# jafarinia/snuffy

Measured on AMD Instinct MI355X. Metric: slides/sec, higher is better.
Workload: dtype f32; 1 GPU; cfgB: MILNet eval forward, 1 bag/step/rank, N=32768 patches D=768 h=6 Lambda=200 (K=200) depth=1 relu mlp x4; parallelism=bag-parallel x1, bags_resident_per_rank=8, launch=hip graph replay, rccl_ranks=0

## Files before the change

### include/snuffy_hip.h

```cpp
#ifndef SNUFFY_HIP_H
#define SNUFFY_HIP_H

#include <stddef.h>
#include <stdint.h>

#ifdef __cplusplus
extern "C" {
#endif

typedef void* snf_stream_t;

#define SNF_OK 0
#define SNF_EINVAL (-1)
#define SNF_ELAUNCH (-2)
#define SNF_EUNSUPPORTED (-3)
#define SNF_EWORKSPACE (-4)

#define SNF_ACT_RELU 0
#define SNF_ACT_GELU 1
#define SNF_ACT_LEAKYRELU 2
#define SNF_ACT_SELU 3
#define SNF_ACT_NONE 4

#define SNF_DT_F32 0
// ... 171 lines not shown
int snf_gemm_bf16_resid_f32(const void* a, int64_t lda, const void* w, int64_t ldw, const float* bias, const float* resid, int64_t ldr,
                            int64_t m, int n, int k, int act, float* c, int64_t ldc, int tile_n, snf_stream_t stream);
int snf_gemm_bf16_lnfold(const void* a, int64_t lda, const void* w, int64_t ldw, const float* colsum, const float* bias,
                         const float* rowstats, int64_t m, int n, int k, int act, void* c, int64_t ldc, snf_stream_t stream);
int snf_gemm_bf16_resid(const void* a, int64_t lda, const void* w, int64_t ldw, const float* bias, int64_t m, int n, int k, float* x,
                        int64_t ldx, void* x_bf16, int64_t ldxb, float* stats_part, snf_stream_t stream);
int snf_gemm_hl_bf16(const void* a_hl, int64_t lda, const void* w_hl, int64_t ldw, const float* bias, int64_t m, int n, int k,
                     int act, void* c, int64_t ldc, int out_dtype, snf_stream_t stream);
int snf_gemm_hl_resid_bf16(const void* a_hl, int64_t lda, const void* w_hl, int64_t ldw, const float* bias, const float* resid,
                           int64_t ldr, int64_t m, int n, int k, int act, void* c, int64_t ldc, int out_dtype, snf_stream_t stream);
size_t snf_gemm_hl_ws_bytes(int64_t m, int n, int k);
int snf_gemm_hl_gated_bf16(const void* a_hl, int64_t lda, const void* w_hl, int64_t ldw, const void* gate_hl, int64_t ldg, int64_t m, int n,
                           int k, void* c_hl, int64_t ldc, snf_stream_t stream);
size_t snf_gemm_tn_ws_bytes(int64_t n, int p, int q);
int snf_gemm_tn_f32(const void* a, int64_t lda, int a_hi, int a_lo, const void* b, int64_t ldb, int b_hi, int b_lo, int hl, int64_t n, int p,
                    int q, float* c, int64_t ldc, void* workspace, size_t workspace_bytes, snf_stream_t stream);
int snf_gemm_hl_ws_bf16(const void* a_hl, int64_t lda, const void* w_hl, int64_t ldw, const float* bias, const float* resid,
                        int64_t ldr, int64_t m, int n, int k, int act, void* c, int64_t ldc, int out_dtype, void* workspace,
                        size_t workspace_bytes, snf_stream_t stream);
size_t snf_gemm_hl_deferred_ws_bytes(int64_t m, int n, int k, size_t* slab_offset);
int snf_gemm_hl_deferred_f32(const void* a_hl, int64_t lda, const void* w_hl, int64_t ldw, const float* bias, const float* resid,
                             int64_t ldr, int64_t m, int n, int k, int act, float* c, int64_t ldc, int out_dtype, void* workspace,
                             size_t workspace_bytes, snf_stream_t stream);
int snf_gemm_hl_dropout_bf16(const void* a_hl, int64_t lda, const void* w_hl, int64_t ldw, const float* bias, const float* resid,
                             int64_t ldr, int64_t m, int n, int k, int act, void* c, int64_t ldc, int out_dtype, float dropout_p,
                             uint64_t seed, uint64_t offset, snf_stream_t stream);
int snf_gemm_hl_ws_dropout_bf16(const void* a_hl, int64_t lda, const void* w_hl, int64_t ldw, const float* bias, const float* resid,
                                int64_t ldr, int64_t m, int n, int k, int act, void* c, int64_t ldc, int out_dtype, float dropout_p,
                                uint64_t seed, uint64_t offset, void* workspace, size_t workspace_bytes, snf_stream_t stream);
int snf_split_hl_colsum_dropout_f32(const float* x, int64_t ldx, int64_t m, int k, const void* gate_hl, int64_t ldg, float dropout_p,
                                    uint64_t seed, uint64_t offset, void* out_hl, int64_t ldo, float* partial, snf_stream_t stream);
int snf_split_hl_f32(const float* x, int64_t ldx, int64_t m, int k, void* out_bf16, snf_stream_t stream);
int snf_layernorm_rows_hl_f32(const float* x, int64_t n, int d, const int32_t* slot_map, const float* patch_rows,
                              const float* gamma, const float* beta, float eps, void* out_bf16, snf_stream_t stream);
int snf_layernorm_rows_hl_patch_f32(const float* x, const float* addend, int64_t n, int d, const int64_t* out_row_idx,
                                    const float* gamma, const float* beta, float eps, void* out_hl, snf_stream_t stream);

int snf_vit_patchify(const float* img, int b, int c, int hgt, int wid, int patch, void* cols, int out_dtype,
                     snf_stream_t stream);
int snf_vit_assemble_tokens(const void* patch_emb, int pe_dtype, const float* cls_token, const float* pos_embed, int b,
                            int num_patches, int d, float* tokens, snf_stream_t stream);
int snf_vit_residual_ln(float* x, int64_t n, int d, const void* add1_bf16, const void* add2_bf16, float scale2,
                        const float* gamma, const float* beta, float eps, void* ln_out_bf16, void* x_bf16,
                        snf_stream_t stream);
int snf_vit_row_stats(const float* x, int64_t ldx, const float* part, int slots, int64_t n, int d, float eps, float* stats,
                      void* x_bf16, int64_t ldxb, snf_stream_t stream);
// ... 140 lines not shown
```

### snuffy_amd/_ffi.py

```python
import ctypes
import os
from ctypes import c_char_p, c_float, c_int, c_int64, c_size_t, c_uint64, c_void_p

_HERE = os.path.dirname(os.path.abspath(__file__))
LIB_PATH = os.environ.get("SNUFFY_HIP_LIB") or os.path.join(_HERE, "lib", "libsnuffy_hip.so")

SNF_OK = 0
SNF_EINVAL = -1
SNF_ELAUNCH = -2
SNF_EUNSUPPORTED = -3
SNF_EWORKSPACE = -4

ACT_CODES = {"relu": 0, "gelu": 1, "leakyrelu": 2, "selu": 3, "none": 4}
DT_F32 = 0
DT_BF16 = 1
DT_BF16_SPLIT3 = 2
DT_BF16_HL = 3
TOPK_MAX_K = 2048

SIGNATURES = {
    "snf_version": (c_char_p, []),
    "snf_last_error": (c_char_p, []),
    "snf_device_cu_count": (c_int, []),
    "snf_critic_f32": (c_int, [c_void_p, c_int64, c_int, c_void_p, c_void_p, c_int, c_void_p, c_void_p, c_void_p,
# ... 111 lines not shown
                                     c_void_p, c_int64, c_void_p]),
    "snf_gemm_bf16_resid": (c_int, [c_void_p, c_int64, c_void_p, c_int64, c_void_p, c_int64, c_int, c_int, c_void_p, c_int64, c_void_p,
                                    c_int64, c_void_p, c_void_p]),
    "snf_vit_row_stats": (c_int, [c_void_p, c_int64, c_void_p, c_int, c_int64, c_int, c_float, c_void_p, c_void_p, c_int64, c_void_p]),
    "snf_split_hl_f32": (c_int, [c_void_p, c_int64, c_int64, c_int, c_void_p, c_void_p]),
    "snf_layernorm_rows_hl_patch_f32": (c_int, [c_void_p, c_void_p, c_int64, c_int, c_void_p, c_void_p, c_void_p, c_float, c_void_p,
                                                c_void_p]),
    "snf_layernorm_rows_hl_f32": (c_int, [c_void_p, c_int64, c_int, c_void_p, c_void_p, c_void_p, c_void_p, c_float,
                                          c_void_p, c_void_p]),
    "snf_gemm_hl_resid_bf16": (c_int, [c_void_p, c_int64, c_void_p, c_int64, c_void_p, c_void_p, c_int64, c_int64, c_int, c_int, c_int,
                                       c_void_p, c_int64, c_int, c_void_p]),
    "snf_gemm_hl_ws_bytes": (c_size_t, [c_int64, c_int, c_int]),
    "snf_gemm_hl_gated_bf16": (c_int, [c_void_p, c_int64, c_void_p, c_int64, c_void_p, c_int64, c_int64, c_int, c_int, c_void_p, c_int64,
                                       c_void_p]),
    "snf_gemm_tn_ws_bytes": (c_size_t, [c_int64, c_int, c_int]),
    "snf_gemm_tn_f32": (c_int, [c_void_p, c_int64, c_int, c_int, c_void_p, c_int64, c_int, c_int, c_int, c_int64, c_int, c_int, c_void_p,
                                c_int64, c_void_p, c_size_t, c_void_p]),
    "snf_split_hl_colsum_f32": (c_int, [c_void_p, c_int64, c_int64, c_int, c_void_p, c_int64, c_void_p, c_int64, c_void_p, c_void_p]),
    "snf_gemm_hl_ws_bf16": (c_int, [c_void_p, c_int64, c_void_p, c_int64, c_void_p, c_void_p, c_int64, c_int64, c_int, c_int, c_int,
                                    c_void_p, c_int64, c_int, c_void_p, c_size_t, c_void_p]),
    "snf_gemm_hl_deferred_ws_bytes": (c_size_t, [c_int64, c_int, c_int, c_void_p]),
    "snf_gemm_hl_deferred_f32": (c_int, [c_void_p, c_int64, c_void_p, c_int64, c_void_p, c_void_p, c_int64, c_int64, c_int, c_int, c_int,
                                         c_void_p, c_int64, c_int, c_void_p, c_size_t, c_void_p]),
    "snf_gemm_bf16_dropout": (c_int, [c_void_p, c_int64, c_void_p, c_int64, c_void_p, c_int64, c_int, c_int, c_int, c_void_p, c_int64,
                                      c_int, c_int, c_float, c_uint64, c_uint64, c_void_p]),
    "snf_dropout_rows_bf16": (c_int, [c_void_p, c_int64, c_int64, c_int, c_float, c_uint64, c_uint64, c_void_p]),
    "snf_residual_assemble_dropout_f32": (c_int, [c_void_p, c_int64, c_int, c_void_p, c_void_p, c_void_p, c_void_p, c_float, c_uint64,
                                                  c_uint64, c_void_p, c_void_p]),
    "snf_colsum_fused_dropout": (c_int, [c_void_p, c_int, c_int64, c_int, c_float, c_uint64, c_uint64, c_void_p, c_void_p, c_void_p]),
    "snf_gemm_hl_dropout_bf16": (c_int, [c_void_p, c_int64, c_void_p, c_int64, c_void_p, c_void_p, c_int64, c_int64, c_int, c_int, c_int,
                                         c_void_p, c_int64, c_int, c_float, c_uint64, c_uint64, c_void_p]),
    "snf_gemm_hl_ws_dropout_bf16": (c_int, [c_void_p, c_int64, c_void_p, c_int64, c_void_p, c_void_p, c_int64, c_int64, c_int, c_int, c_int,
                                            c_void_p, c_int64, c_int, c_float, c_uint64, c_uint64, c_void_p, c_size_t, c_void_p]),
    "snf_split_hl_colsum_dropout_f32": (c_int, [c_void_p, c_int64, c_int64, c_int, c_void_p, c_int64, c_float, c_uint64, c_uint64,
                                                c_void_p, c_int64, c_void_p, c_void_p]),
    "snf_gemm_hl_bf16": (c_int, [c_void_p, c_int64, c_void_p, c_int64, c_void_p, c_int64, c_int, c_int, c_int, c_void_p, c_int64,
                                 c_int, c_void_p]),
    "snf_topk_segmented_f32": (c_int, [c_void_p, c_void_p, c_int, c_int64, c_int, c_void_p, c_void_p]),
    "snf_sparse_attn_varlen_plan": (c_int, [c_void_p, c_int, c_int, c_int, c_int, c_void_p, c_size_t, c_void_p, c_void_p]),
    "snf_sparse_attn_fwd_mfma_varlen": (c_int, [c_void_p, c_int64, c_void_p, c_int64, c_void_p, c_int, c_void_p, c_int, c_int, c_int,
                                                c_int, c_float, c_void_p, c_void_p, c_void_p, c_void_p, c_void_p, c_size_t,
                                                c_void_p]),
    "snf_sparse_attn_x3_varlen_plan": (c_int, [c_void_p, c_int, c_int, c_int, c_int, c_void_p, c_size_t, c_void_p, c_void_p]),
    "snf_sparse_attn_fwd_x3_varlen": (c_int, [c_void_p, c_int64, c_void_p, c_int64, c_void_p, c_void_p, c_int, c_int, c_int, c_int,
                                              c_float, c_void_p, c_void_p, c_void_p, c_void_p, c_void_p, c_size_t, c_void_p]),
    "snf_sparse_attn_varlen_chunked_plan": (c_int, [c_void_p, c_int, c_int, c_int, c_int, c_void_p, c_size_t, c_void_p, c_void_p,
# ... 105 lines not shown
```

### snuffy_amd/csrc/gemm.hip

```cpp
#include <stdlib.h>

#include "mfma.h"
#include "philox.h"

namespace {

struct GemmParams {
    const unsigned short* a;
    const unsigned short* w;
    const float* bias;
    void* c;
    int64_t lda, ldw, ldc;
    int m, n, k;
    int act;
    int tiles_m, tiles_n;
    unsigned long long* trace;
    const float* resid = nullptr;
    int64_t ldr = 0;
    unsigned int* split_cnt = nullptr;
    float* split_slab = nullptr;
    int split_cap = 0, split_rcap = 0;
    const unsigned short* gate = nullptr;
    int64_t ldg = 0;
    const float* colsum = nullptr;
// ... 436 lines not shown
            barrier();
        }
        bias_landed();
#ifdef SNF_GEMM_NOSTORE
        if (false) {
#else
        if (full) {
#endif
            epilogue(tile, std::true_type{});
            after_epilogue = true;
        } else {
            epilogue(tile, std::false_type{});
            wait_vmcnt<0>();
        }
        if (!has_next) break;
        tile = next;
        cur = nxt;
    }
    if (wid < 4) __builtin_amdgcn_s_barrier();
}

template <int ACT, int OUT, int SPLIT_MODE = 0, bool GATE = false, bool DROP = false>
__global__ __launch_bounds__(512, 2) void gemm_hl_kernel(GemmParams P) {
    constexpr bool SPLIT = SPLIT_MODE != 0, DEFER = SPLIT_MODE == 2;
    static_assert(!DEFER || (SPLIT && OUT == 1 && ACT == SNF_ACT_NONE && !GATE && !DROP), "gemm_hl: the deferred split writes plain fp32");
    static_assert(!GATE || (OUT == 3 && ACT == SNF_ACT_NONE && !SPLIT), "gemm_hl: the gated form writes an hl image, no activation, no split");
    static_assert(!DROP || (!GATE && (OUT == 1 || OUT == 3)), "gemm_hl: dropout goes with the fp32 and the hl-image outputs");
    constexpr int NI = 4, BN = 256;
    constexpr int ROWL = 128;
    constexpr int IMG = BM * ROWL;
    constexpr int STEP_BYTES = 2 * IMG;
    constexpr int NC = 4 * NI;
    constexpr bool LINE_STORES = (OUT == 1 || OUT == 3) && ACT != SNF_ACT_GELU && ACT != SNF_ACT_SELU;
    extern __shared__ __attribute__((aligned(16))) unsigned char smem[];

    const int lane = threadIdx.x & 63;
    const int wid = __builtin_amdgcn_readfirstlane(threadIdx.x >> 6);
    const int wr = wid >> 2, wc = wid & 3;
    const int ns_all = P.k / BKS;
    unsigned char* const scr = smem + 2 * STEP_BYTES + wid * 4096;

    const int ntiles = P.tiles_m * P.tiles_n;
    const int xcd = blockIdx.x & 7, wg_in_xcd = blockIdx.x >> 3, wgs_per_xcd = gridDim.x >> 3;
    if constexpr (!SPLIT) {
        if (P.split_cap >= 2 && blockIdx.x == 0) {
            for (int i = threadIdx.x; i < 8 * P.split_rcap; i += 512) P.split_cnt[i] = 0u;
            asm volatile("s_waitcnt vmcnt(0)" ::: "memory");
        }
    }
    int t_lo, t_hi;
    {
        const int q = ntiles >> 3, r = ntiles & 7;
        t_lo = xcd < r ? xcd * (q + 1) : r * (q + 1) + (xcd - r) * q;
        t_hi = t_lo + q + (xcd < r ? 1 : 0);
    }
    int sp_part = 0, sp_parts = 1, sp_slot = 0, sp_tile = -1;
    if (P.split_cap >= 2) {
        const int q_x = t_hi - t_lo, full_rounds = q_x / wgs_per_xcd, r = q_x - full_rounds * wgs_per_xcd;
        int sn = r > 0 ? wgs_per_xcd / r : 0;
        if (sn > P.split_cap) sn = P.split_cap;
        if (sn > ns_all / HL_SPLIT_MIN_STEPS) sn = ns_all / HL_SPLIT_MIN_STEPS;
        if (sn >= 2 && r <= P.split_rcap) {
            if constexpr (SPLIT) {
                if (wg_in_xcd < r * sn) {
                    const int jr = wg_in_xcd % r;
                    sp_tile = t_lo + full_rounds * wgs_per_xcd + jr;
                    sp_part = wg_in_xcd / r, sp_parts = sn, sp_slot = xcd * P.split_rcap + jr;
                }
            } else {
                t_hi = t_lo + full_rounds * wgs_per_xcd;
            }
        }
    }
    int tile = t_lo + wg_in_xcd;
    if constexpr (SPLIT) {
        tile = __builtin_amdgcn_readfirstlane(sp_tile);
        sp_part = __builtin_amdgcn_readfirstlane(sp_part), sp_parts = __builtin_amdgcn_readfirstlane(sp_parts);
        sp_slot = __builtin_amdgcn_readfirstlane(sp_slot);
        if (tile < 0) return;
        t_hi = tile + 1;
        asm volatile("" : "+s"(t_hi));
    } else {
        if (tile >= t_hi) return;
    }
    const int s_begin = SPLIT ? __builtin_amdgcn_readfirstlane(sp_part * ns_all / sp_parts) : 0;
    const int ns = SPLIT ? __builtin_amdgcn_readfirstlane((sp_part + 1) * ns_all / sp_parts) - s_begin : ns_all;
    const unsigned short* const a_base = P.a + (SPLIT ? s_begin * 64 : 0);
    const unsigned short* const w_base = P.w + (SPLIT ? s_begin * 64 : 0);

    struct Src {
        int a[4], w[4];
    };
    auto tile_src_mn = [&](int tm, int tn) __attribute__((always_inline)) -> Src {
        Src s;
        int ln = lane;
        asm volatile("" : "+v"(ln));
        const int c = ln & 7;
#pragma unroll
        for (int j = 0; j < 4; ++j) {
            const int row = (4 * wid + j) * 8 + (ln >> 3);
            int grow = tm * BM + row;
            if (grow > P.m - 1) grow = P.m - 1;
            s.a[j] = grow * (int)P.lda + ((c ^ ((row >> 1) & 7)) << 3);
            int wrow = tn * BN + row;
            if (wrow > P.n - 1) wrow = P.n - 1;
            s.w[j] = wrow * (int)P.ldw + ((c ^ (((row >> 1) & 1) | (((row >> 3) & 3) << 1))) << 3);
        }
        return s;
    };
// ... 21 lines not shown

    f32x4 acc[8][NI];
    bf16x8 xf[8], wh[NI], wl[NI];
    f32x4 bv4[NC / 4];

    auto frag = [&](const unsigned char* p) __attribute__((always_inline)) -> bf16x8 {
#ifdef X3_NOREAD
        u32x4 z = {1u, 2u, 3u, (unsigned)lane};
        asm volatile("" : "+v"(z));
        return __builtin_bit_cast(bf16x8, z);
#endif
        return __builtin_bit_cast(bf16x8, *reinterpret_cast<const u32x4*>(p));
    };
#ifdef X3_NOMFMA
#define X3_MFMA(a, b, c) ([&]() { f32x4 t_ = (c); asm volatile("" : "+v"(t_) : "v"(a), "v"(b)); return t_; }())
#else
#define X3_MFMA(a, b, c) __builtin_amdgcn_mfma_f32_16x16x32_bf16(a, b, c, 0, 0, 0)
#endif
    auto load_bias = [&](int tl) __attribute__((always_inline)) {
#pragma unroll
        for (int c4 = 0; c4 < NC / 4; ++c4) bv4[c4] = f32x4{0.f, 0.f, 0.f, 0.f};
        if (P.bias) {
            const int tn = tl % P.tiles_n;
            const int n0 = tn * BN + 64 * wc + 8 * fg;
            const float* bp0 = P.bias + (n0 + 8 <= P.n ? n0 : 0);
            const float* bp1 = P.bias + (n0 + 40 <= P.n ? n0 + 32 : 0);
            asm volatile("global_load_dwordx4 %0, %1, off" : "=v"(bv4[0]) : "v"(bp0) : "memory");
            asm volatile("global_load_dwordx4 %0, %1, off offset:16" : "=v"(bv4[1]) : "v"(bp0) : "memory");
            asm volatile("global_load_dwordx4 %0, %1, off" : "=v"(bv4[2]) : "v"(bp1) : "memory");
            asm volatile("global_load_dwordx4 %0, %1, off offset:16" : "=v"(bv4[3]) : "v"(bp1) : "memory");
        }
    };
    auto bias_landed = [&]() __attribute__((always_inline)) {
#pragma unroll
        for (int c4 = 0; c4 < NC / 4; ++c4) asm volatile("" : "+v"(bv4[c4]));
    };
    auto epilogue = [&](int tl, auto full_t) __attribute__((always_inline)) {
        constexpr bool FULL = decltype(full_t)::value;
        const int tm = tl / P.tiles_n, tn = tl - tm * P.tiles_n;
        const int n0 = tn * BN + 64 * wc + 8 * fg;
        const int row0 = tm * BM + 128 * wr + fi;
        int lane_o = lane;
        asm volatile("" : "+v"(lane_o));
        const int fio = lane_o & 15, fgo = lane_o >> 4;
#pragma unroll
        for (int mi = 0; mi < 8; ++mi) {
            const int row = row0 + 16 * mi;
#pragma unroll
            for (int h = 0; h < NI / 2; ++h) {
                float v[8];
#pragma unroll
                for (int e = 0; e < 8; ++e) v[e] = activate<ACT>(acc[mi][2 * h + (e >> 2)][e & 3] + bv4[2 * h + (e >> 2)][e & 3]);
                const int col = n0 + 32 * h;
                if constexpr (DROP) {
                    const snf::philox_f4 m0 = snf::dropout_mask4(P.drop, 0, P.m, row, P.n, col);
                    const snf::philox_f4 m1 = snf::dropout_mask4(P.drop, 0, P.m, row, P.n, col + 4);
#pragma unroll
                    for (int e = 0; e < 4; ++e) {
                        v[e] *= m0[e];
                        v[4 + e] *= m1[e];
                    }
#pragma unroll
                    for (int e = 0; e < 8; ++e) asm volatile("" : "+v"(v[e]));
                }
// ... 36 lines not shown
                        if (ok) *reinterpret_cast<u32x4*>(dst) = pk;
                    } else {
                        float lo[8];
#pragma unroll
                        for (int e = 0; e < 8; ++e)
                            lo[e] = v[e] - __uint_as_float((e & 1) ? (pk[e >> 1] & 0xffff0000u) : (pk[e >> 1] << 16));
                        const u32x4 pl = {cvt_pk_bf16(lo[0], lo[1]), cvt_pk_bf16(lo[2], lo[3]), cvt_pk_bf16(lo[4], lo[5]), cvt_pk_bf16(lo[6], lo[7])};
                        unsigned short* dst = reinterpret_cast<unsigned short*>(P.c) + (int64_t)row * P.ldc + 64 * (col >> 5) + (col & 31);
                        if constexpr (LINE_STORES) {
                            *reinterpret_cast<u32x4*>(scr + fio * 256 + (((8 * h + fgo) ^ fio) << 4)) = pk;
                            *reinterpret_cast<u32x4*>(scr + fio * 256 + (((8 * h + 4 + fgo) ^ fio) << 4)) = pl;
                        } else if (ok) {
                            *reinterpret_cast<u32x4*>(dst) = pk;
                            *reinterpret_cast<u32x4*>(dst + 32) = pl;
                        }
                    }
                }
            }
            if constexpr (LINE_STORES) {
                const int lr = lane_o >> 4, lc = lane_o & 15;
                unsigned char* const crow = reinterpret_cast<unsigned char*>(P.c) +
                                            (OUT == 1 ? 4 * (int64_t)(tn * BN + 64 * wc) : 2 * 2 * (int64_t)(tn * BN + 64 * wc));
                const int64_t pitch = (OUT == 1 ? 4 : 2) * P.ldc;
#pragma unroll
                for (int jj = 0; jj < 4; ++jj) {
                    const int r = lr + 4 * jj;
                    const u32x4 val = *reinterpret_cast<const u32x4*>(scr + r * 256 + ((lc ^ r) << 4));
                    const int orow = tm * BM + 128 * wr + 16 * mi + r;
                    const int ocol = tn * BN + 64 * wc + (OUT == 1 ? 4 * lc : 32 * (lc >> 3) + 8 * (lc & 3));
#ifdef X3_NOSTORE
                    const bool ok2 = val[0] == 0x12345678u && orow < 0;
#else
                    const bool ok2 = FULL || (orow < P.m && ocol + (OUT == 1 ? 4 : 8) <= P.n);
#endif
                    if (ok2) *reinterpret_cast<u32x4*>(crow + orow * pitch + 16 * lc) = val;
                }
            }
        }
    };

    Src cur = tile_src(tile);
    stage(cur, 0, 0);
    int buf = 0;
    bool after_epilogue = false;
    while (true) {
        const int next = tile + wgs_per_xcd;
        const bool has_next = next < t_hi;
        const bool full = (tile / P.tiles_n + 1) * BM <= P.m && (tile % P.tiles_n + 1) * BN <= P.n;
        for (int s = 0; s < ns; ++s) {
            if (!(s == 0 && after_epilogue)) wait_vmcnt<0>();
            after_epilogue = false;
            __builtin_amdgcn_sched_barrier(0);
            __builtin_amdgcn_s_barrier();
            __builtin_amdgcn_sched_barrier(0);
            const unsigned char* base = smem + buf * STEP_BYTES;
#pragma unroll
            for (int ni = 0; ni < NI; ++ni) wh[ni] = frag(base + woff_h + (4 * (ni & 1) + 32 * (ni >> 1)) * ROWL);
#pragma unroll
            for (int mi = 0; mi < 8; ++mi) xf[mi] = frag(base + xoff_h + mi * 16 * ROWL);
#pragma unroll
            for (int ni = 0; ni < NI; ++ni) wl[ni] = frag(base + woff_l + (4 * (ni & 1) + 32 * (ni >> 1)) * ROWL);
            __builtin_amdgcn_sched_barrier(0);
            if (s + 1 < ns) {
                stage(cur, s + 1, buf ^ 1);
            } else if (has_next) {
                cur = tile_src(next);
                stage(cur, 0, buf ^ 1);
            }
            __builtin_amdgcn_sched_barrier(0);
            __builtin_amdgcn_s_setprio(1);
            if (s == 0) {
#pragma unroll
                for (int mi = 0; mi < 8; ++mi)
#pragma unroll
                    for (int ni = 0; ni < NI; ++ni) acc[mi][ni] = X3_MFMA(wh[ni], xf[mi], (f32x4{0.f, 0.f, 0.f, 0.f}));
            } else {
#pragma unroll
                for (int mi = 0; mi < 8; ++mi)
#pragma unroll
                    for (int ni = 0; ni < NI; ++ni) acc[mi][ni] = X3_MFMA(wh[ni], xf[mi], acc[mi][ni]);
            }
#pragma unroll
            for (int mi = 0; mi < 8; ++mi) {
#pragma unroll
                for (int ni = 0; ni < NI; ++ni) acc[mi][ni] = X3_MFMA(wl[ni], xf[mi], acc[mi][ni]);
                __builtin_amdgcn_sched_barrier(0);
                xf[mi] = frag(base + xoff_l + mi * 16 * ROWL);
                __builtin_amdgcn_sched_barrier(0);
            }
#pragma unroll
            for (int mi = 0; mi < 8; ++mi)
#pragma unroll
                for (int ni = 0; ni < NI; ++ni) acc[mi][ni] = X3_MFMA(wh[ni], xf[mi], acc[mi][ni]);
            __builtin_amdgcn_s_setprio(0);
            buf ^= 1;
        }
        int etile = tile;
        bool efull = full;
#ifdef SNF_GEMM_SPLIT_NOSUM
        if constexpr (false) {
#else
        if constexpr (DEFER) {
            if (sp_part != 0) {
                int mark = sp_slot + 1;
                asm volatile("" : "+s"(mark));
                if (threadIdx.x == 0) reinterpret_cast<int*>(P.split_cnt)[tile] = mark;
                P.c = P.split_slab + (size_t)sp_slot * (size_t)(BM * BN);
                P.ldc = BN;
                P.bias = nullptr, P.resid = nullptr;
                etile = 0, efull = true;
            }
        } else if constexpr (SPLIT) {
#endif
            volatile unsigned int& s_ticket = *reinterpret_cast<volatile unsigned int*>(smem);
            float* slab0 = P.split_slab + (size_t)sp_slot * P.split_cap * (size_t)(BM * BN);
            unsigned tix = threadIdx.x;
            asm volatile("" : "+v"(tix));
            f32x4* mine = reinterpret_cast<f32x4*>(slab0 + (size_t)sp_part * (BM * BN)) + tix;
            wait_vmcnt<0>();
#pragma unroll
            for (int mi = 0; mi < 8; ++mi)
#pragma unroll
                for (int ni = 0; ni < NI; ++ni) mine[(mi * NI + ni) * 512] = acc[mi][ni];
            wait_vmcnt<0>();
            __syncthreads();
            if (tix == 0) {
// ... 12 lines not shown
#pragma unroll
            for (int mi = 0; mi < 8; ++mi)
#pragma unroll
                for (int ni = 0; ni < NI; ++ni) {
                    f32x4 sum = {0.f, 0.f, 0.f, 0.f};
                    for (int pp = 0; pp < sp_parts; ++pp) {
                        f32x4 v = acc[mi][ni];
                        if (pp != sp_part) v = reinterpret_cast<const f32x4*>(slab0 + (size_t)pp * (BM * BN))[(mi * NI + ni) * 512 + tix];
                        sum = pp == 0 ? v : sum + v;
                    }
                    acc[mi][ni] = sum;
                }
        }
        load_bias(etile);
        wait_vmcnt<0>();
        bias_landed();
        if (efull)
            epilogue(etile, std::true_type{});
        else
            epilogue(etile, std::false_type{});
        after_epilogue = true;
        if (!has_next) break;
        tile = next;
    }
}

template <int ACT, int OUT, bool DROP = false>
int launch_hl(const GemmParams& P, hipStream_t s) {
    constexpr int lds = 2 * 2 * BM * 128 + (((OUT == 1 || OUT == 3) && ACT != SNF_ACT_GELU && ACT != SNF_ACT_SELU) ? 8 * 4096 : 0);
    auto kern = [] {
        if constexpr (DROP) return gemm_hl_kernel<ACT, OUT, false, false, true>;
        else return gemm_hl_kernel<ACT, OUT>;
    }();
    static thread_local unsigned long long attr_set_mask = 0;
    if (int rc = snf::lds_opt_in(reinterpret_cast<const void*>(kern), lds, &attr_set_mask, "gemm_hl")) return rc;
    const int ntiles = P.tiles_m * P.tiles_n;
    int grid = snf::cu_count() & ~7;
    if (grid < 8) grid = 8;
    {
        static const int dbg_grid = getenv("SNF_GEMM_HL_GRID") ? atoi(getenv("SNF_GEMM_HL_GRID")) & ~7 : 0;
        if (dbg_grid >= 8 && dbg_grid < grid && P.split_cap < 2) grid = dbg_grid;
    }
    const int per_xcd = (ntiles + 7) / 8;
    if (per_xcd * 8 < grid) grid = per_xcd * 8;
    hipLaunchKernelGGL(kern, dim3(grid), dim3(512), lds, s, P);
    int rc = snf::check_launch("gemm_hl_kernel");
// ... 466 lines not shown
        P.drop = *drop;
        if (hl_out && act == SNF_ACT_RELU && !resid) return launch_hl<SNF_ACT_RELU, 3, true>(P, s);
        if (out_dtype == SNF_DT_F32 && act == SNF_ACT_NONE) return launch_hl<SNF_ACT_NONE, 1, true>(P, s);
        snf::set_error("snf_gemm_hl_dropout_bf16: dropout exists for act = relu with an hl-image output and for act = none with an fp32 "
                       "output (got act %d, out_dtype %d)", act, out_dtype);
        return SNF_EUNSUPPORTED;
    }
    if (hl_out) return launch_hl_act<3>(P, s);
    return out_dtype == SNF_DT_F32 ? launch_hl_act<1>(P, s) : launch_hl_act<0>(P, s);
}
}

extern "C" int snf_gemm_hl_ws_bf16(const void* a_hl, int64_t lda, const void* w_hl, int64_t ldw, const float* bias,
                                   const float* resid, int64_t ldr, int64_t m, int n, int k, int act, void* c, int64_t ldc,
                                   int out_dtype, void* workspace, size_t workspace_bytes, snf_stream_t stream) {
    return gemm_hl_ws_impl(a_hl, lda, w_hl, ldw, bias, resid, ldr, m, n, k, act, c, ldc, out_dtype, nullptr, workspace, workspace_bytes, stream);
}

namespace {
struct HlDeferred {
    HlSplit g;
    int map_rcap;
    size_t slab_offset, bytes;
};
HlDeferred hl_deferred_geometry(int64_t m, int n, int k) {
    HlDeferred d = {hl_split_geometry(m, n, k), 0, 0, 0};
    if (d.g.cap < 2) return d;
    d.g.cap = 2;
    const int ntiles = (int)(((m + BM - 1) / BM) * ((n + 255) / 256));
    d.map_rcap = (ntiles + 7) / 8 > d.g.rcap ? (ntiles + 7) / 8 : d.g.rcap;
    d.slab_offset = ((size_t)8 * d.map_rcap * sizeof(int32_t) + 4095) & ~(size_t)4095;
    d.bytes = d.slab_offset + (size_t)8 * d.g.rcap * (size_t)(BM * 256) * sizeof(float);
    return d;
}

int launch_hl_deferred(GemmParams P, const HlDeferred& d, hipStream_t s) {
    constexpr int lds = 2 * 2 * BM * 128 + 8 * 4096;
    auto kern = gemm_hl_kernel<SNF_ACT_NONE, 1>;
    auto kern2 = gemm_hl_kernel<SNF_ACT_NONE, 1, 2>;
    static thread_local unsigned long long attr_set_mask = 0, attr_set2_mask = 0;
    if (int rc = snf::lds_opt_in(reinterpret_cast<const void*>(kern), lds, &attr_set_mask, "gemm_hl")) return rc;
    if (int rc = snf::lds_opt_in(reinterpret_cast<const void*>(kern2), lds, &attr_set2_mask, "gemm_hl")) return rc;
    const int ntiles = P.tiles_m * P.tiles_n;
    int grid = snf::cu_count() & ~7;
    if (grid < 8) grid = 8;
    const int per_xcd = (ntiles + 7) / 8;
    if (per_xcd * 8 < grid) grid = per_xcd * 8;
    P.split_cap = 2, P.split_rcap = d.map_rcap;
    hipLaunchKernelGGL(kern, dim3(grid), dim3(512), lds, s, P);
    if (int rc = snf::check_launch("gemm_hl_kernel")) return rc;
    P.split_rcap = d.g.rcap;
    hipLaunchKernelGGL(kern2, dim3(grid), dim3(512), lds, s, P);
    return snf::check_launch("gemm_hl_kernel<deferred split>");
}
}

extern "C" size_t snf_gemm_hl_deferred_ws_bytes(int64_t m, int n, int k, size_t* slab_offset) {
    const HlDeferred d = hl_deferred_geometry(m, n, k);
    if (slab_offset) *slab_offset = d.slab_offset;
    return d.bytes;
}

extern "C" int snf_gemm_hl_deferred_f32(const void* a_hl, int64_t lda, const void* w_hl, int64_t ldw, const float* bias, const float* resid,
                                        int64_t ldr, int64_t m, int n, int k, int act, float* c, int64_t ldc, int out_dtype, void* workspace,
                                        size_t workspace_bytes, snf_stream_t stream) {
    SNF_REQUIRE(a_hl && w_hl && c && workspace, "snf_gemm_hl_deferred_f32: null pointer");
    SNF_REQUIRE(m >= 1 && n >= 1 && k >= 1, "snf_gemm_hl_deferred_f32: bad shape m=%lld n=%d k=%d", (long long)m, n, k);
    if (act != SNF_ACT_NONE || out_dtype != SNF_DT_F32) {
        snf::set_error("snf_gemm_hl_deferred_f32: fp32 output without activation only (act %d, out_dtype %d)", act, out_dtype);
        return SNF_EUNSUPPORTED;
    }
    SNF_REQUIRE(!resid || (ldr >= n && ldr % 4 == 0 && reinterpret_cast<uintptr_t>(resid) % 16 == 0),
                "snf_gemm_hl_deferred_f32: a residual needs 16-byte aligned rows (ldr=%lld)", (long long)ldr);
    const HlDeferred d = hl_deferred_geometry(m, n, k);
    if (k % BKS || k < BKS || n % 8 || lda % 8 || ldw % 8 || ldc % 4 || lda < 2 * (int64_t)k || ldw < 2 * (int64_t)k || ldc < n ||
        (reinterpret_cast<uintptr_t>(a_hl) | reinterpret_cast<uintptr_t>(w_hl) | reinterpret_cast<uintptr_t>(c)) % 16 ||
        (bias && reinterpret_cast<uintptr_t>(bias) % 16) || m * lda >= 0x7fffffffll || (int64_t)n * ldw >= 0x7fffffffll || !d.bytes) {
        snf::set_error("snf_gemm_hl_deferred_f32: shape m=%lld n=%d k=%d (lda %lld ldw %lld ldc %lld) outside the kernel's domain "
                       "(snf_gemm_hl_bf16's, and a last round that splits: snf_gemm_hl_deferred_ws_bytes > 0)",
                       (long long)m, n, k, (long long)lda, (long long)ldw, (long long)ldc);
        return SNF_EUNSUPPORTED;
    }
    if (workspace_bytes < d.bytes || reinterpret_cast<uintptr_t>(workspace) % 128) {
        snf::set_error("snf_gemm_hl_deferred_f32: workspace %zu < %zu (or not 128-byte aligned)", workspace_bytes, d.bytes);
        return SNF_EWORKSPACE;
    }
    GemmParams P;
    P.a = reinterpret_cast<const unsigned short*>(a_hl);
    P.w = reinterpret_cast<const unsigned short*>(w_hl);
    P.bias = bias;
    P.c = c;
    P.lda = lda, P.ldw = ldw, P.ldc = ldc;
    P.m = (int)m, P.n = n, P.k = k, P.act = act;
    P.tiles_m = (int)((m + BM - 1) / BM);
    P.tiles_n = (n + 255) / 256;
    P.trace = nullptr;
    P.resid = resid;
    P.ldr = ldr;
    P.split_cnt = reinterpret_cast<unsigned int*>(workspace);
    P.split_slab = reinterpret_cast<float*>(reinterpret_cast<unsigned char*>(workspace) + d.slab_offset);
    return launch_hl_deferred(P, d, snf::as_stream(stream));
}

extern "C" int snf_gemm_hl_ws_dropout_bf16(const void* a_hl, int64_t lda, const void* w_hl, int64_t ldw, const float* bias,
                                           const float* resid, int64_t ldr, int64_t m, int n, int k, int act, void* c, int64_t ldc,
                                           int out_dtype, float dropout_p, uint64_t seed, uint64_t offset, void* workspace,
                                           size_t workspace_bytes, snf_stream_t stream) {
    SNF_REQUIRE(dropout_p >= 0.f && dropout_p < 1.f, "snf_gemm_hl_dropout_bf16: dropout_p=%f outside [0, 1)", dropout_p);
    const snf::DropoutState st = snf::make_dropout(dropout_p, seed, offset);
    return gemm_hl_ws_impl(a_hl, lda, w_hl, ldw, bias, resid, ldr, m, n, k, act, c, ldc, out_dtype, &st, workspace, workspace_bytes, stream);
}

extern "C" int snf_gemm_hl_dropout_bf16(const void* a_hl, int64_t lda, const void* w_hl, int64_t ldw, const float* bias,
                                        const float* resid, int64_t ldr, int64_t m, int n, int k, int act, void* c, int64_t ldc,
                                        int out_dtype, float dropout_p, uint64_t seed, uint64_t offset, snf_stream_t stream) {
    return snf_gemm_hl_ws_dropout_bf16(a_hl, lda, w_hl, ldw, bias, resid, ldr, m, n, k, act, c, ldc, out_dtype, dropout_p, seed, offset,
                                       nullptr, 0, stream);
}

extern "C" int snf_gemm_hl_gated_bf16(const void* a_hl, int64_t lda, const void* w_hl, int64_t ldw, const void* gate_hl, int64_t ldg, int64_t m,
                                      int n, int k, void* c_hl, int64_t ldc, snf_stream_t stream) {
    SNF_REQUIRE(a_hl && w_hl && gate_hl && c_hl, "snf_gemm_hl_gated_bf16: null pointer");
    SNF_REQUIRE(m >= 1 && n >= 1 && k >= 1, "snf_gemm_hl_gated_bf16: bad shape m=%lld n=%d k=%d", (long long)m, n, k);
    if (k % BKS || k < BKS || n % 32 || lda % 8 || ldw % 8 || ldc % 8 || ldg % 8 || lda < 2 * (int64_t)k || ldw < 2 * (int64_t)k ||
// ... 57 lines not shown
```

### snuffy_amd/ops.py

```python
import collections
import ctypes
import math

import torch

from . import _ffi
from ._ffi import ACT_CODES, DT_BF16, DT_BF16_HL, DT_BF16_SPLIT3, DT_F32, TOPK_MAX_K, check


def _p(t):
    return None if t is None else ctypes.c_void_p(t.data_ptr())


_raw_stream = getattr(torch._C, "_cuda_getCurrentRawStream", None)


def _stream():
    if _raw_stream is not None:
        return ctypes.c_void_p(_raw_stream(torch.cuda.current_device()))
    return ctypes.c_void_p(torch.cuda.current_stream().cuda_stream)


def _on_current_device(t, name):
    if t.device.index != torch.cuda.current_device():
# ... 1618 lines not shown


def gemm_hl_gated(a_hl, w_hl, gate_hl):
    a_hl, w_hl, gate_hl = _rows16(a_hl, "a_hl"), _rows16(w_hl, "w_hl"), _rows16(gate_hl, "gate_hl")
    if a_hl.dtype != torch.bfloat16 or w_hl.dtype != torch.bfloat16 or gate_hl.dtype != torch.bfloat16:
        raise TypeError("gemm_hl_gated: operands must be bfloat16 hl images")
    m, k2 = a_hl.shape
    n = w_hl.shape[0]
    if w_hl.shape[1] != k2 or k2 % 64 or n % 32 or tuple(gate_hl.shape) != (m, 2 * n):
        raise ValueError("gemm_hl_gated: inconsistent shapes")
    out = torch.empty(m, 2 * n, dtype=torch.bfloat16, device=a_hl.device)
    check(_ffi.load().snf_gemm_hl_gated_bf16(_p(a_hl), a_hl.stride(0), _p(w_hl), w_hl.stride(0), _p(gate_hl), gate_hl.stride(0), m, n,
                                             k2 // 2, _p(out), out.stride(0), _stream()), "snf_gemm_hl_gated_bf16")
    return out


def hl_colsum(img):
    s, _ = colsum_fused(img)
    return s.view(-1, 2, 32).sum(1).reshape(-1)


GEMM_HL_SPLITK = True
GEMM_HL_DEFERRED = True


class DeferredK:

    __slots__ = ("slabs", "tile_map", "ws")

    def __init__(self, slabs, tile_map, ws):
        self.slabs, self.tile_map, self.ws = slabs, tile_map, ws

    def add_to(self, z):
        z = z.clone()
        for tm, tn in self.tile_map.nonzero().tolist():
            blk = z[256 * tm:256 * (tm + 1), 256 * tn:256 * (tn + 1)]
            blk += self.slabs[int(self.tile_map[tm, tn]) - 1, :blk.shape[0], :blk.shape[1]]
        return z


def gemm_hl_deferred_ws_bytes(m, n, k):
    return int(_ffi.load().snf_gemm_hl_deferred_ws_bytes(m, n, k, None))


def gemm_hl_deferred(a_hl, w_hl, bias=None, resid=None, workspace=None):
    if a_hl.dtype != torch.bfloat16 or w_hl.dtype != torch.bfloat16:
        raise TypeError("gemm_hl_deferred: operands must be bfloat16 hl images")
    a_hl = _rows16(a_hl, "a_hl")
    w_hl = _rows16(w_hl, "w_hl")
    m, k2 = a_hl.shape
    n = w_hl.shape[0]
    if w_hl.shape[1] != k2 or k2 % 64:
        raise ValueError("gemm_hl_deferred: images are %s and %s" % (tuple(a_hl.shape), tuple(w_hl.shape)))
    if bias is not None:
        bias = _req(bias, torch.float32, "bias", 1)
    ldr = 0
    if resid is not None:
        if resid.dtype != torch.float32 or tuple(resid.shape) != (m, n):
            raise ValueError("gemm_hl_deferred: resid needs an fp32 [m, n] tensor")
        resid = _rows16(resid, "resid")
        ldr = resid.stride(0)
    lib = _ffi.load()
    off = ctypes.c_size_t(0)
    ws_bytes = int(lib.snf_gemm_hl_deferred_ws_bytes(m, n, k2 // 2, ctypes.byref(off)))
    if not ws_bytes:
        raise ValueError("gemm_hl_deferred: m=%d n=%d k=%d has no split last round" % (m, n, k2 // 2))
    ws = workspace
    if ws is None:
        ws = torch.empty(ws_bytes, dtype=torch.uint8, device=a_hl.device)
    elif ws.dtype != torch.uint8 or ws.dim() != 1 or not ws.is_contiguous() or ws.numel() < ws_bytes or ws.device != a_hl.device:
        raise ValueError("gemm_hl_deferred: workspace must be a contiguous uint8 tensor of >= %d bytes on %s" % (ws_bytes, a_hl.device))
    out = torch.empty(m, n, dtype=torch.float32, device=a_hl.device)
    check(lib.snf_gemm_hl_deferred_f32(_p(a_hl), a_hl.stride(0), _p(w_hl), w_hl.stride(0), _p(bias), _p(resid), ldr, m, n, k2 // 2,
                                       ACT_CODES["none"], _p(out), out.stride(0), DT_F32, _p(ws), ws_bytes, _stream()),
          "snf_gemm_hl_deferred_f32")
    tm, tn = (m + 255) // 256, (n + 255) // 256
    tile_map = ws[:4 * tm * tn].view(torch.int32).view(tm, tn)
    slabs = ws[off.value:ws_bytes].view(torch.float32).view(-1, 256, 256)
    return out, DeferredK(slabs, tile_map, ws)


def _hl_workspace(device, nbytes):
    return _ws(nbytes, device)


def split3_weight(w, colscale=None):
    w = w.detach().float()
    if colscale is not None:
        colscale = colscale.detach().float().contiguous()
    if w.is_cuda and w.dim() == 2 and w.shape[1] % 8 == 0 and w.stride(1) == 1 and w.stride(0) % 4 == 0 and w.data_ptr() % 16 == 0:
        out = torch.empty(w.shape[0], 3 * w.shape[1], dtype=torch.bfloat16, device=w.device)
        check(_ffi.load().snf_split3_weight_f32(_p(w), w.stride(0), w.shape[0], w.shape[1], _p(colscale), _p(out), _stream()),
              "snf_split3_weight_f32")
        return out
    if colscale is not None:
        w = w * colscale
    hi = w.to(torch.bfloat16)
    lo = (w - hi.float()).to(torch.bfloat16)
# ... 441 lines not shown
```

### snuffy_amd/snuffy.py

```python
import copy
import math

import numpy as np
import torch
import torch.nn as nn

from . import functional as SF
from . import ops

device = torch.device("cuda" if torch.cuda.is_available() else "cpu")


class RuntimeConfig:

    def __init__(self, precision="fp32", return_attention=True):
        self.stack = None
        self.sampler = "reference"
        self._device_sampler = None
        self._draws = 0
        self.set(precision, return_attention)

    def set_sampler(self, sampler):
        if sampler not in ("reference", "device"):
            raise ValueError("sampler must be 'reference' or 'device', got %r" % (sampler,))
# ... 248 lines not shown
        feats, classes = self._critic(x)
        prediction_bag, A = self.b_classifier(feats, classes)
        return classes, prediction_bag, A

    _GRAPH_SHAPES = 1024
    _GRAPH_COPY_BYTES = 32 << 20

    def _graph_ok(self, x):
        lim = getattr(self, "_graph_max_patches", 0)
        if lim <= 0 or self.training or torch.is_grad_enabled():
            return False
        if not (isinstance(x, torch.Tensor) and x.is_cuda and x.dim() == 3 and x.shape[0] == 1 and x.dtype == torch.float32
                and x.is_contiguous() and 0 < x.shape[1] <= lim and type(self.i_classifier) is FCLayer):
            return False
        if self.b_classifier.cfg.return_attention and x.numel() * 4 > self._GRAPH_COPY_BYTES:
            return False
        on_device = self.b_classifier.cfg.sampler == "device"
        return all(type(l) is EncoderLayer and (l.random_patch_share == 0 or on_device) for l in self.b_classifier.encoder.layers)

    def _weights_signature(self):
        plist = list(self.parameters())
        knobs = tuple((l.big_lambda, l.random_patch_share) for l in self.b_classifier.encoder.layers)
        knobs += (SF.FP32_GEMM, SF.FP32_ATTENTION, SF.X3_HL_ATTENTION, SF.X3_HL_KPFRAG, SF.X3_HL_KPFRAG_GATHER, SF.FP32_SHARED_NORM, ops.GEMM_HL_SPLITK, ops.GEMM_HL_DEFERRED,
                  SF.BF16_DEEP_STACKS, self.b_classifier.cfg.sampler)
        return tuple(SF.param_key(p) for p in plist), knobs

    def invalidate(self):
        if getattr(self, "_graph_max_patches", 0):
            self._graphs.clear()
            self._graph_seen.clear()
            self._graph_sig = None
        for layer in self.b_classifier.encoder.layers:
            SF.invalidate_folded(layer)
        SF.drop_param_caches(self)
        return self

    _GRAPH_STATE = ("_graphs", "_graph_seen", "_graph_pool", "_graph_sig", "_packed_bags", "_capture_stream")

    def __deepcopy__(self, memo):
        new = self.__class__.__new__(self.__class__)
        memo[id(self)] = new
        for k, v in self.__dict__.items():
            if k not in self._GRAPH_STATE:
                new.__dict__[k] = copy.deepcopy(v, memo)
        if getattr(self, "_graph_max_patches", 0):
            new._graphs, new._graph_seen, new._graph_pool = {}, set(), None
        new.b_classifier.cfg._device_sampler = None
# ... 103 lines not shown
```

Measured before the change: 921.0 slides/s.

## Fuse deferred split-K GEMM into a single persistent launch

Adds a one-launch variant of the deferred split-K hl GEMM. Each workgroup first runs its full tiles, then picks up its split-K part of a remainder tile, writing the tile map and partial slabs in the same kernel instead of a second launch. The intent is to remove a kernel launch and its tail/drain gap inside the graph. It adds geometry checks that fall back to the two-launch path, and more register pressure from extra per-lane state.

```diff
diff --git a/include/snuffy_hip.h b/include/snuffy_hip.h
--- a/include/snuffy_hip.h
+++ b/include/snuffy_hip.h
@@ -217,6 +217,9 @@
 int snf_gemm_hl_deferred_f32(const void* a_hl, int64_t lda, const void* w_hl, int64_t ldw, const float* bias, const float* resid,
                              int64_t ldr, int64_t m, int n, int k, int act, float* c, int64_t ldc, int out_dtype, void* workspace,
                              size_t workspace_bytes, snf_stream_t stream);
+int snf_gemm_hl_deferred_one_f32(const void* a_hl, int64_t lda, const void* w_hl, int64_t ldw, const float* bias, const float* resid,
+                                 int64_t ldr, int64_t m, int n, int k, int act, float* c, int64_t ldc, int out_dtype, void* workspace,
+                                 size_t workspace_bytes, snf_stream_t stream);
 int snf_gemm_hl_dropout_bf16(const void* a_hl, int64_t lda, const void* w_hl, int64_t ldw, const float* bias, const float* resid,
                              int64_t ldr, int64_t m, int n, int k, int act, void* c, int64_t ldc, int out_dtype, float dropout_p,
                              uint64_t seed, uint64_t offset, snf_stream_t stream);
diff --git a/snuffy_amd/_ffi.py b/snuffy_amd/_ffi.py
--- a/snuffy_amd/_ffi.py
+++ b/snuffy_amd/_ffi.py
@@ -157,6 +157,8 @@
     "snf_gemm_hl_deferred_ws_bytes": (c_size_t, [c_int64, c_int, c_int, c_void_p]),
     "snf_gemm_hl_deferred_f32": (c_int, [c_void_p, c_int64, c_void_p, c_int64, c_void_p, c_void_p, c_int64, c_int64, c_int, c_int, c_int,
                                          c_void_p, c_int64, c_int, c_void_p, c_size_t, c_void_p]),
+    "snf_gemm_hl_deferred_one_f32": (c_int, [c_void_p, c_int64, c_void_p, c_int64, c_void_p, c_void_p, c_int64, c_int64, c_int, c_int, c_int,
+                                             c_void_p, c_int64, c_int, c_void_p, c_size_t, c_void_p]),
     "snf_gemm_bf16_dropout": (c_int, [c_void_p, c_int64, c_void_p, c_int64, c_void_p, c_int64, c_int, c_int, c_int, c_void_p, c_int64,
                                       c_int, c_int, c_float, c_uint64, c_uint64, c_void_p]),
     "snf_dropout_rows_bf16": (c_int, [c_void_p, c_int64, c_int64, c_int, c_float, c_uint64, c_uint64, c_void_p]),
diff --git a/snuffy_amd/csrc/gemm.hip b/snuffy_amd/csrc/gemm.hip
--- a/snuffy_amd/csrc/gemm.hip
+++ b/snuffy_amd/csrc/gemm.hip
@@ -482,8 +482,9 @@
 
 template <int ACT, int OUT, int SPLIT_MODE = 0, bool GATE = false, bool DROP = false>
 __global__ __launch_bounds__(512, 2) void gemm_hl_kernel(GemmParams P) {
-    constexpr bool SPLIT = SPLIT_MODE != 0, DEFER = SPLIT_MODE == 2;
+    constexpr bool SPLIT = SPLIT_MODE == 1 || SPLIT_MODE == 2, DEFER = SPLIT_MODE == 2, ONE = SPLIT_MODE == 3;
     static_assert(!DEFER || (SPLIT && OUT == 1 && ACT == SNF_ACT_NONE && !GATE && !DROP), "gemm_hl: the deferred split writes plain fp32");
+    static_assert(!ONE || (OUT == 1 && ACT == SNF_ACT_NONE && !GATE && !DROP), "gemm_hl: the one-launch deferred split writes plain fp32");
     static_assert(!GATE || (OUT == 3 && ACT == SNF_ACT_NONE && !SPLIT), "gemm_hl: the gated form writes an hl image, no activation, no split");
     static_assert(!DROP || (!GATE && (OUT == 1 || OUT == 3)), "gemm_hl: dropout goes with the fp32 and the hl-image outputs");
     constexpr int NI = 4, BN = 256;
@@ -502,7 +503,7 @@
 
     const int ntiles = P.tiles_m * P.tiles_n;
     const int xcd = blockIdx.x & 7, wg_in_xcd = blockIdx.x >> 3, wgs_per_xcd = gridDim.x >> 3;
-    if constexpr (!SPLIT) {
+    if constexpr (!SPLIT && !ONE) {
         if (P.split_cap >= 2 && blockIdx.x == 0) {
             for (int i = threadIdx.x; i < 8 * P.split_rcap; i += 512) P.split_cnt[i] = 0u;
             asm volatile("s_waitcnt vmcnt(0)" ::: "memory");
@@ -521,19 +522,26 @@
         if (sn > P.split_cap) sn = P.split_cap;
         if (sn > ns_all / HL_SPLIT_MIN_STEPS) sn = ns_all / HL_SPLIT_MIN_STEPS;
         if (sn >= 2 && r <= P.split_rcap) {
-            if constexpr (SPLIT) {
+            if constexpr (SPLIT || ONE) {
                 if (wg_in_xcd < r * sn) {
                     const int jr = wg_in_xcd % r;
                     sp_tile = t_lo + full_rounds * wgs_per_xcd + jr;
                     sp_part = wg_in_xcd / r, sp_parts = sn, sp_slot = xcd * P.split_rcap + jr;
                 }
-            } else {
-                t_hi = t_lo + full_rounds * wgs_per_xcd;
-            }
+            }
+            if constexpr (!SPLIT) t_hi = t_lo + full_rounds * wgs_per_xcd;
         }
     }
     int tile = t_lo + wg_in_xcd;
-    if constexpr (SPLIT) {
+    int p_begin = 0, p_ns = 0;
+    if constexpr (ONE) {
+        sp_tile = __builtin_amdgcn_readfirstlane(sp_tile), sp_slot = __builtin_amdgcn_readfirstlane(sp_slot);
+        sp_part = __builtin_amdgcn_readfirstlane(sp_part), sp_parts = __builtin_amdgcn_readfirstlane(sp_parts);
+        t_hi = __builtin_amdgcn_readfirstlane(t_hi);
+        p_begin = __builtin_amdgcn_readfirstlane(sp_part * ns_all / sp_parts);
+        p_ns = __builtin_amdgcn_readfirstlane((sp_part + 1) * ns_all / sp_parts) - p_begin;
+        if (tile >= t_hi) return;
+    } else if constexpr (SPLIT) {
         tile = __builtin_amdgcn_readfirstlane(sp_tile);
         sp_part = __builtin_amdgcn_readfirstlane(sp_part), sp_parts = __builtin_amdgcn_readfirstlane(sp_parts);
         sp_slot = __builtin_amdgcn_readfirstlane(sp_slot);
@@ -544,7 +552,7 @@
         if (tile >= t_hi) return;
     }
     const int s_begin = SPLIT ? __builtin_amdgcn_readfirstlane(sp_part * ns_all / sp_parts) : 0;
-    const int ns = SPLIT ? __builtin_amdgcn_readfirstlane((sp_part + 1) * ns_all / sp_parts) - s_begin : ns_all;
+    int ns = SPLIT ? __builtin_amdgcn_readfirstlane((sp_part + 1) * ns_all / sp_parts) - s_begin : ns_all;
     const unsigned short* const a_base = P.a + (SPLIT ? s_begin * 64 : 0);
     const unsigned short* const w_base = P.w + (SPLIT ? s_begin * 64 : 0);
 
@@ -612,7 +620,13 @@
         for (int c4 = 0; c4 < NC / 4; ++c4) bv4[c4] = f32x4{0.f, 0.f, 0.f, 0.f};
         if (P.bias) {
             const int tn = tl % P.tiles_n;
-            const int n0 = tn * BN + 64 * wc + 8 * fg;
+            int fgb = fg;
+            if constexpr (ONE) {
+                int ln = lane;
+                asm volatile("" : "+v"(ln));
+                fgb = ln >> 4;
+            }
+            const int n0 = tn * BN + 64 * wc + 8 * fgb;
             const float* bp0 = P.bias + (n0 + 8 <= P.n ? n0 : 0);
             const float* bp1 = P.bias + (n0 + 40 <= P.n ? n0 + 32 : 0);
             asm volatile("global_load_dwordx4 %0, %1, off" : "=v"(bv4[0]) : "v"(bp0) : "memory");
@@ -628,8 +642,10 @@
     auto epilogue = [&](int tl, auto full_t) __attribute__((always_inline)) {
         constexpr bool FULL = decltype(full_t)::value;
         const int tm = tl / P.tiles_n, tn = tl - tm * P.tiles_n;
-        const int n0 = tn * BN + 64 * wc + 8 * fg;
-        const int row0 = tm * BM + 128 * wr + fi;
+        int lane_e = lane;
+        if constexpr (ONE) asm volatile("" : "+v"(lane_e));
+        const int n0 = tn * BN + 64 * wc + 8 * (ONE ? lane_e >> 4 : fg);
+        const int row0 = tm * BM + 128 * wr + (ONE ? lane_e & 15 : fi);
         int lane_o = lane;
         asm volatile("" : "+v"(lane_o));
         const int fio = lane_o & 15, fgo = lane_o >> 4;
@@ -712,6 +728,8 @@
                 unsigned char* const crow = reinterpret_cast<unsigned char*>(P.c) +
                                             (OUT == 1 ? 4 * (int64_t)(tn * BN + 64 * wc) : 2 * 2 * (int64_t)(tn * BN + 64 * wc));
                 const int64_t pitch = (OUT == 1 ? 4 : 2) * P.ldc;
+                int lc16 = 16 * lc;
+                if constexpr (ONE) asm volatile("" : "+v"(lc16));
 #pragma unroll
                 for (int jj = 0; jj < 4; ++jj) {
                     const int r = lr + 4 * jj;
@@ -723,7 +741,7 @@
 #else
                     const bool ok2 = FULL || (orow < P.m && ocol + (OUT == 1 ? 4 : 8) <= P.n);
 #endif
-                    if (ok2) *reinterpret_cast<u32x4*>(crow + orow * pitch + 16 * lc) = val;
+                    if (ok2) *reinterpret_cast<u32x4*>(crow + orow * pitch + lc16) = val;
                 }
             }
         }
@@ -733,9 +751,20 @@
     stage(cur, 0, 0);
     int buf = 0;
     bool after_epilogue = false;
+    bool in_part = false;
     while (true) {
-        const int next = tile + wgs_per_xcd;
-        const bool has_next = next < t_hi;
+        int next = tile + wgs_per_xcd;
+        bool has_next = next < t_hi;
+        int next_k = 0;
+        bool to_part = false;
+        if constexpr (ONE) {
+            if (in_part) {
+                has_next = false;
+            } else if (!has_next && sp_tile >= 0) {
+                has_next = to_part = true;
+                next = sp_tile, next_k = p_begin * 64;
+            }
+        }
         const bool full = (tile / P.tiles_n + 1) * BM <= P.m && (tile % P.tiles_n + 1) * BN <= P.n;
         for (int s = 0; s < ns; ++s) {
             if (!(s == 0 && after_epilogue)) wait_vmcnt<0>();
@@ -755,6 +784,10 @@
                 stage(cur, s + 1, buf ^ 1);
             } else if (has_next) {
                 cur = tile_src(next);
+                if constexpr (ONE) {
+#pragma unroll
+                    for (int j = 0; j < 4; ++j) cur.a[j] += next_k, cur.w[j] += next_k;
+                }
                 stage(cur, 0, buf ^ 1);
             }
             __builtin_amdgcn_sched_barrier(0);
@@ -787,11 +820,14 @@
         }
         int etile = tile;
         bool efull = full;
+        if constexpr (ONE) {
+            if (!in_part && threadIdx.x == 0) reinterpret_cast<int*>(P.split_cnt)[tile] = 0;
+        }
 #ifdef SNF_GEMM_SPLIT_NOSUM
         if constexpr (false) {
 #else
-        if constexpr (DEFER) {
-            if (sp_part != 0) {
+        if constexpr (DEFER || ONE) {
+            if (sp_part != 0 && (DEFER || in_part)) {
                 int mark = sp_slot + 1;
                 asm volatile("" : "+s"(mark));
                 if (threadIdx.x == 0) reinterpret_cast<int*>(P.split_cnt)[tile] = mark;
@@ -850,6 +886,9 @@
         after_epilogue = true;
         if (!has_next) break;
         tile = next;
+        if constexpr (ONE) {
+            if (to_part) in_part = true, ns = p_ns;
+        }
     }
 }
 
@@ -1362,30 +1401,47 @@
     HlSplit g;
     int map_rcap;
     size_t slab_offset, bytes;
+    bool one_launch;
 };
 HlDeferred hl_deferred_geometry(int64_t m, int n, int k) {
-    HlDeferred d = {hl_split_geometry(m, n, k), 0, 0, 0};
+    HlDeferred d = {hl_split_geometry(m, n, k), 0, 0, 0, false};
     if (d.g.cap < 2) return d;
     d.g.cap = 2;
     const int ntiles = (int)(((m + BM - 1) / BM) * ((n + 255) / 256));
     d.map_rcap = (ntiles + 7) / 8 > d.g.rcap ? (ntiles + 7) / 8 : d.g.rcap;
     d.slab_offset = ((size_t)8 * d.map_rcap * sizeof(int32_t) + 4095) & ~(size_t)4095;
     d.bytes = d.slab_offset + (size_t)8 * d.g.rcap * (size_t)(BM * 256) * sizeof(float);
+    int grid = snf::cu_count() & ~7;
+    if (grid < 8) grid = 8;
+    if ((ntiles + 7) / 8 * 8 < grid) grid = (ntiles + 7) / 8 * 8;
+    const int w = grid >> 3;
+    d.one_launch = true;
+    for (int x = 0; x < 8; ++x) {
+        const int q = ntiles / 8 + (x < (ntiles & 7) ? 1 : 0), r = q % w;
+        if (r && w / r >= 2 && k / BKS / HL_SPLIT_MIN_STEPS >= 2 && q < w) d.one_launch = false;
+    }
     return d;
 }
 
-int launch_hl_deferred(GemmParams P, const HlDeferred& d, hipStream_t s) {
+int launch_hl_deferred(GemmParams P, const HlDeferred& d, bool one, hipStream_t s) {
     constexpr int lds = 2 * 2 * BM * 128 + 8 * 4096;
     auto kern = gemm_hl_kernel<SNF_ACT_NONE, 1>;
     auto kern2 = gemm_hl_kernel<SNF_ACT_NONE, 1, 2>;
-    static thread_local unsigned long long attr_set_mask = 0, attr_set2_mask = 0;
+    auto kern1 = gemm_hl_kernel<SNF_ACT_NONE, 1, 3>;
+    static thread_local unsigned long long attr_set_mask = 0, attr_set2_mask = 0, attr_set1_mask = 0;
     if (int rc = snf::lds_opt_in(reinterpret_cast<const void*>(kern), lds, &attr_set_mask, "gemm_hl")) return rc;
     if (int rc = snf::lds_opt_in(reinterpret_cast<const void*>(kern2), lds, &attr_set2_mask, "gemm_hl")) return rc;
+    if (int rc = snf::lds_opt_in(reinterpret_cast<const void*>(kern1), lds, &attr_set1_mask, "gemm_hl")) return rc;
     const int ntiles = P.tiles_m * P.tiles_n;
     int grid = snf::cu_count() & ~7;
     if (grid < 8) grid = 8;
     const int per_xcd = (ntiles + 7) / 8;
     if (per_xcd * 8 < grid) grid = per_xcd * 8;
+    if (one && d.one_launch) {
+        P.split_cap = 2, P.split_rcap = d.g.rcap;
+        hipLaunchKernelGGL(kern1, dim3(grid), dim3(512), lds, s, P);
+        return snf::check_launch("gemm_hl_kernel<deferred split, one launch>");
+    }
     P.split_cap = 2, P.split_rcap = d.map_rcap;
     hipLaunchKernelGGL(kern, dim3(grid), dim3(512), lds, s, P);
     if (int rc = snf::check_launch("gemm_hl_kernel")) return rc;
@@ -1401,9 +1457,10 @@
     return d.bytes;
 }
 
-extern "C" int snf_gemm_hl_deferred_f32(const void* a_hl, int64_t lda, const void* w_hl, int64_t ldw, const float* bias, const float* resid,
-                                        int64_t ldr, int64_t m, int n, int k, int act, float* c, int64_t ldc, int out_dtype, void* workspace,
-                                        size_t workspace_bytes, snf_stream_t stream) {
+namespace {
+int gemm_hl_deferred_impl(const void* a_hl, int64_t lda, const void* w_hl, int64_t ldw, const float* bias, const float* resid, int64_t ldr,
+                          int64_t m, int n, int k, int act, float* c, int64_t ldc, int out_dtype, void* workspace, size_t workspace_bytes,
+                          bool one, snf_stream_t stream) {
     SNF_REQUIRE(a_hl && w_hl && c && workspace, "snf_gemm_hl_deferred_f32: null pointer");
     SNF_REQUIRE(m >= 1 && n >= 1 && k >= 1, "snf_gemm_hl_deferred_f32: bad shape m=%lld n=%d k=%d", (long long)m, n, k);
     if (act != SNF_ACT_NONE || out_dtype != SNF_DT_F32) {
@@ -1439,7 +1496,20 @@
     P.ldr = ldr;
     P.split_cnt = reinterpret_cast<unsigned int*>(workspace);
     P.split_slab = reinterpret_cast<float*>(reinterpret_cast<unsigned char*>(workspace) + d.slab_offset);
-    return launch_hl_deferred(P, d, snf::as_stream(stream));
+    return launch_hl_deferred(P, d, one, snf::as_stream(stream));
+}
+}
+
+extern "C" int snf_gemm_hl_deferred_f32(const void* a_hl, int64_t lda, const void* w_hl, int64_t ldw, const float* bias, const float* resid,
+                                        int64_t ldr, int64_t m, int n, int k, int act, float* c, int64_t ldc, int out_dtype, void* workspace,
+                                        size_t workspace_bytes, snf_stream_t stream) {
+    return gemm_hl_deferred_impl(a_hl, lda, w_hl, ldw, bias, resid, ldr, m, n, k, act, c, ldc, out_dtype, workspace, workspace_bytes, false, stream);
+}
+
+extern "C" int snf_gemm_hl_deferred_one_f32(const void* a_hl, int64_t lda, const void* w_hl, int64_t ldw, const float* bias, const float* resid,
+                                            int64_t ldr, int64_t m, int n, int k, int act, float* c, int64_t ldc, int out_dtype, void* workspace,
+                                            size_t workspace_bytes, snf_stream_t stream) {
+    return gemm_hl_deferred_impl(a_hl, lda, w_hl, ldw, bias, resid, ldr, m, n, k, act, c, ldc, out_dtype, workspace, workspace_bytes, true, stream);
 }
 
 extern "C" int snf_gemm_hl_ws_dropout_bf16(const void* a_hl, int64_t lda, const void* w_hl, int64_t ldw, const float* bias,
diff --git a/snuffy_amd/ops.py b/snuffy_amd/ops.py
--- a/snuffy_amd/ops.py
+++ b/snuffy_amd/ops.py
@@ -1664,6 +1664,7 @@
 
 GEMM_HL_SPLITK = True
 GEMM_HL_DEFERRED = True
+GEMM_HL_DEFERRED_ONE_LAUNCH = True
 
 
 class DeferredK:
@@ -1685,7 +1686,7 @@
     return int(_ffi.load().snf_gemm_hl_deferred_ws_bytes(m, n, k, None))
 
 
-def gemm_hl_deferred(a_hl, w_hl, bias=None, resid=None, workspace=None):
+def gemm_hl_deferred(a_hl, w_hl, bias=None, resid=None, workspace=None, one_launch=None):
     if a_hl.dtype != torch.bfloat16 or w_hl.dtype != torch.bfloat16:
         raise TypeError("gemm_hl_deferred: operands must be bfloat16 hl images")
     a_hl = _rows16(a_hl, "a_hl")
@@ -1713,9 +1714,9 @@
     elif ws.dtype != torch.uint8 or ws.dim() != 1 or not ws.is_contiguous() or ws.numel() < ws_bytes or ws.device != a_hl.device:
         raise ValueError("gemm_hl_deferred: workspace must be a contiguous uint8 tensor of >= %d bytes on %s" % (ws_bytes, a_hl.device))
     out = torch.empty(m, n, dtype=torch.float32, device=a_hl.device)
-    check(lib.snf_gemm_hl_deferred_f32(_p(a_hl), a_hl.stride(0), _p(w_hl), w_hl.stride(0), _p(bias), _p(resid), ldr, m, n, k2 // 2,
-                                       ACT_CODES["none"], _p(out), out.stride(0), DT_F32, _p(ws), ws_bytes, _stream()),
-          "snf_gemm_hl_deferred_f32")
+    name = "snf_gemm_hl_deferred_one_f32" if (GEMM_HL_DEFERRED_ONE_LAUNCH if one_launch is None else one_launch) else "snf_gemm_hl_deferred_f32"
+    check(getattr(lib, name)(_p(a_hl), a_hl.stride(0), _p(w_hl), w_hl.stride(0), _p(bias), _p(resid), ldr, m, n, k2 // 2,
+                             ACT_CODES["none"], _p(out), out.stride(0), DT_F32, _p(ws), ws_bytes, _stream()), name)
     tm, tn = (m + 255) // 256, (n + 255) // 256
     tile_map = ws[:4 * tm * tn].view(torch.int32).view(tm, tn)
     slabs = ws[off.value:ws_bytes].view(torch.float32).view(-1, 256, 256)
diff --git a/snuffy_amd/snuffy.py b/snuffy_amd/snuffy.py
--- a/snuffy_amd/snuffy.py
+++ b/snuffy_amd/snuffy.py
@@ -294,7 +294,7 @@
         plist = list(self.parameters())
         knobs = tuple((l.big_lambda, l.random_patch_share) for l in self.b_classifier.encoder.layers)
         knobs += (SF.FP32_GEMM, SF.FP32_ATTENTION, SF.X3_HL_ATTENTION, SF.X3_HL_KPFRAG, SF.X3_HL_KPFRAG_GATHER, SF.FP32_SHARED_NORM, ops.GEMM_HL_SPLITK, ops.GEMM_HL_DEFERRED,
-                  SF.BF16_DEEP_STACKS, self.b_classifier.cfg.sampler)
+                  ops.GEMM_HL_DEFERRED_ONE_LAUNCH, SF.BF16_DEEP_STACKS, self.b_classifier.cfg.sampler)
         return tuple(SF.param_key(p) for p in plist), knobs
 
     def invalidate(self):
```

Result: no change. 928.3 slides/s, median of 6 (+0.8%).
